# greatscottgadgets/libbtbb

Measured on AMD Instinct MI355X. Metric: Gbit/s raw bitstream scanned (LAP_ANY, err<=2), higher is better.
Workload: dtype u64; 1 GPU; promiscuous LAP_ANY scan, 4 GiB packed single-channel synthetic bitstream per GPU, max_ac_errors=2, sync word every 4096 symbols; symbols_per_gpu=34359738305, hits_per_gpu=6402406, parallelism=time-sharded x1 (btbbx_shard_plan: slices + 63-symbol halo), no collectives

## Files before the change

libbtbb_amd/csrc/packet_trials.h:

```cpp
#pragma once


__device__ __forceinline__ uint32_t lds_now(const uint32_t *p)
{
	return *(volatile __attribute__((address_space(3))) const uint32_t *)p;
}

#define TL_THREADS 512
#define TL_PACKETS (TL_THREADS / 16)
#define TL_WGS_PER_CU (1024 / TL_THREADS)
#define TL_TRIALS  (TL_PACKETS * 64)
#define TL_A_BLOCKS 183
#define TL_A_BYTES  232
#define TL_B_BLOCKS 10
#define TL_B_BYTES  16
#ifdef TL_PROFILE
__device__ unsigned long long g_tl_prof[16];
#define TL_PROF_START __shared__ uint32_t tl_acc[16]; if (threadIdx.x < 16) tl_acc[threadIdx.x] = 0; uint64_t tl_t = __builtin_readcyclecounter()
#define TL_PROF(k) do { const uint64_t n_ = __builtin_readcyclecounter(); if (tid == 0) tl_acc[k] += (uint32_t)(n_ - tl_t); tl_t = n_; } while (0)
#define TL_PROF_END do { __syncthreads(); if (tid < 16) atomicAdd(&g_tl_prof[tid], (unsigned long long)tl_acc[tid]); } while (0)
#else
#define TL_PROF_START do { } while (0)
#define TL_PROF(k) do { } while (0)
#define TL_PROF_END do { } while (0)
#endif
#define TL_AFAIL(p) lds_now(&a_fail[p])
__global__ __launch_bounds__(TL_THREADS) __attribute__((amdgpu_waves_per_eu(4, 4))) void trials_linear_kernel(const uint64_t *packets, const btbbx_pkt_in *in,
							     uint32_t n_packets, btbbx_trial *trials, const uint32_t *d_count)
{
	if (d_count)
		n_packets = min(n_packets, *d_count);
	__shared__ uint64_t pk[TL_PACKETS][BTBBX_PKT_WORDS + 1];
	__shared__ __attribute__((aligned(8))) btbbx_pkt_in pin[TL_PACKETS];
	__shared__ uint32_t hdr_ut[TL_PACKETS];
	__shared__ uint16_t clk_ut[64];
	__shared__ __attribute__((aligned(16))) uint16_t pw20[64];
	__shared__ __attribute__((aligned(16))) uint16_t lin[LIN_MAXLEN * 16];
	__shared__ __attribute__((aligned(16))) uint16_t advw[7 * 2 * 256];
	__shared__ uint16_t order[TL_TRIALS];
	__shared__ uint32_t t_info[TL_TRIALS];
	__shared__ int16_t t_rv[TL_TRIALS];
	__shared__ uint32_t pk_sort[TL_PACKETS];
	__shared__ uint32_t type_base[18];
	__shared__ uint16_t a10[TL_PACKETS][TL_A_BLOCKS + 3];
	static_assert(TL_A_BYTES / 4 + LIN_MAXLEN / 4 <= TL_A_BLOCKS + 3, "p4a and p4c of a packet lie in its a10 row");
	__shared__ uint16_t b10[TL_PACKETS][TL_B_BLOCKS + 2];
	__shared__ uint32_t a_bytes[TL_PACKETS][TL_A_BYTES / 4], b_bytes[TL_PACKETS][TL_B_BYTES / 4];
	__shared__ uint32_t a_fail[TL_PACKETS], b_fail[TL_PACKETS];
	__shared__ uint16_t p4b[TL_PACKETS][TL_B_BYTES / 4];
	auto p4a = [&](uint32_t p) { return &a10[p][0]; };
	auto p4c = [&](uint32_t p) { return &a10[p][TL_A_BYTES / 4]; };
	__shared__ int8_t hv_rv[TL_PACKETS];
	__shared__ uint16_t chunk_reg[TL_PACKETS][20];
	const uint32_t tid = threadIdx.x, lane = tid & 63;
	TL_PROF_START;
	for (uint32_t i = tid; i < LIN_MAXLEN * 2; i += TL_THREADS)
		reinterpret_cast<uint4 *>(lin)[i] = reinterpret_cast<const uint4 *>(g_lin)[i];
	for (uint32_t i = tid; i < 7 * 2 * 256 / 8; i += TL_THREADS)
		reinterpret_cast<uint4 *>(advw)[i] = reinterpret_cast<const uint4 *>(g_advw)[i];
	chain_lds_init();
	if (tid >= 64 && tid < 128) {
		const uint32_t wb = (uint32_t)wh_bits(wh_start(tid - 64, 0), 18);
		const uint32_t wt = (wb >> 3) & 0xf;
		uint32_t crank = 0;
		for (uint32_t k = 0; k < 16; k++) {
			const uint64_t mk = __ballot(wt == k);
			if (wt == k)
				crank = __builtin_amdgcn_mbcnt_hi((uint32_t)(mk >> 32), __builtin_amdgcn_mbcnt_lo((uint32_t)mk, 0));
		}
		clk_ut[tid - 64] = (uint16_t)(uap_from_hec(wb & 0x3ff, wb >> 10) | (wt << 8) | (crank << 12));
		const uint32_t v = (uint32_t)wh_bits(wh_start(tid - 64, 18), 7);
		uint32_t x = 0;
		for (int j = 0; j < 7; j++)
			if ((v >> j) & 1)
				x ^= lin[20 * 16 + 8 + j];
		pw20[tid - 64] = (uint16_t)x;
	}
	const uint32_t n_batches = (n_packets + TL_PACKETS - 1) / TL_PACKETS;
	constexpr uint32_t PK_ELEMS = TL_PACKETS * (BTBBX_PKT_WORDS + 1), IN_ELEMS = TL_PACKETS * sizeof(btbbx_pkt_in) / 8;
	constexpr uint32_t PER_THREAD = (PK_ELEMS + IN_ELEMS + TL_THREADS - 1) / TL_THREADS;
	static_assert(sizeof(btbbx_pkt_in) == 16, "two words per btbbx_pkt_in");
	uint64_t pre[PER_THREAD];
	auto fetch = [&](uint32_t b) {
		const uint32_t f = b * TL_PACKETS, have = b < n_batches ? (n_packets - f < TL_PACKETS ? n_packets - f : TL_PACKETS) : 0;
		uint32_t tv = tid;
		asm volatile("" : "+v"(tv));
#pragma unroll
		for (uint32_t k = 0; k < PER_THREAD; k++) {
			const uint32_t i = tv + TL_THREADS * k;
			const uint32_t p = i / (BTBBX_PKT_WORDS + 1), w = i % (BTBBX_PKT_WORDS + 1), e = i - PK_ELEMS;
			const uint64_t *src = packets;
			if (i < PK_ELEMS) {
				if (p < have && w < BTBBX_PKT_WORDS)
					src = packets + (uint64_t)(f + p) * BTBBX_PKT_WORDS + w;
			} else if (e < 2 * have) {
				src = reinterpret_cast<const uint64_t *>(in) + (uint64_t)f * 2 + e;
			}
			pre[k] = *src;
		}
	};
	auto stage_in = [&](uint32_t b) {
		const uint32_t f = b * TL_PACKETS, have = b < n_batches ? (n_packets - f < TL_PACKETS ? n_packets - f : TL_PACKETS) : 0;
		uint32_t tv = tid;
		asm volatile("" : "+v"(tv));
#pragma unroll
		for (uint32_t k = 0; k < PER_THREAD; k++) {
			const uint32_t i = tv + TL_THREADS * k;
			const uint32_t p = i / (BTBBX_PKT_WORDS + 1), w = i % (BTBBX_PKT_WORDS + 1);
			if (i < PK_ELEMS)
				pk[p][w] = (p < have && w < BTBBX_PKT_WORDS) ? pre[k] : 0;
			else if (i < PK_ELEMS + IN_ELEMS)
				reinterpret_cast<uint64_t *>(pin)[i - PK_ELEMS] = pre[k];
		}
		if (tid < TL_PACKETS) {
			a_fail[tid] = TL_A_BLOCKS;
			b_fail[tid] = TL_B_BLOCKS;
		}
	};
	fetch(blockIdx.x);
	stage_in(blockIdx.x);
	fetch(blockIdx.x + gridDim.x);
	for (uint32_t batch = blockIdx.x; batch < n_batches; batch += gridDim.x) {
	const uint32_t first = batch * TL_PACKETS;
	const uint32_t mine = n_packets - first < TL_PACKETS ? n_packets - first : TL_PACKETS;

	__syncthreads();
	TL_PROF(0);

	static_assert(TL_PACKETS <= 64, "one wave ranks the packets of a batch");
	if (tid < 64) {
		const bool live = tid < mine;
		uint32_t h = 0;
		if (live) {
			uint32_t dis;
			const uint32_t hdr = header_fec13(pk[tid], dis);
			h = uap_from_hec(hdr & 0x3ff, hdr >> 10) | (((hdr >> 3) & 0xf) << 8) | ((dis < 4 ? 1u : 0u) << 16);
			hdr_ut[tid] = h;
		}
		const bool fec_ok = (h & 0x10000u) != 0;
		const bool var = live && fec_ok && (pin[live ? tid : 0].flags & F_WHITENED);
		const uint32_t key = !live ? 0u : fec_ok ? (h >> 8) & 0xfu : (uint32_t)pin[tid].type & 0xfu;
		const uint64_t vm = __ballot(var);
		const uint32_t nvar = (uint32_t)__popcll(vm);
		uint32_t rank = __builtin_amdgcn_mbcnt_hi((uint32_t)(vm >> 32), __builtin_amdgcn_mbcnt_lo((uint32_t)vm, 0));
		const bool fixed = live && !var;
		uint32_t cf = 0;
		if (__ballot(fixed)) {
			for (uint32_t k = 0; k < 16; k++) {
				const uint64_t fm = __ballot(fixed && key == k);
				if (fixed && key == k)
					rank = __builtin_amdgcn_mbcnt_hi((uint32_t)(fm >> 32), __builtin_amdgcn_mbcnt_lo((uint32_t)fm, 0));
				if (lane == k)
					cf = (uint32_t)__popcll(fm);
			}
		}
		uint32_t incl = cf;
#pragma unroll
		for (int dd = 1; dd < 16; dd <<= 1) {
			const uint32_t up = __shfl_up(incl, dd);
			if (lane >= (uint32_t)dd)
				incl += up;
		}
		if (lane < 16)
			type_base[lane] = 4u * nvar * lane + 64u * (incl - cf);
		if (lane == 17)
			type_base[17] = nvar;
		if (tid < TL_PACKETS)
			pk_sort[tid] = key | ((var ? 1u : 0u) << 4) | (rank << 8);
	}
	static_assert(TL_THREADS == 16 * TL_PACKETS, "sixteen threads per packet");
	auto a_words = [&](uint32_t p) {
		const uint32_t blocks = TL_AFAIL(p) < TL_A_BLOCKS ? TL_AFAIL(p) : TL_A_BLOCKS, n = (blocks * 10 + 31) / 32 + 1;
		return n < TL_A_BYTES / 4 ? n : (uint32_t)(TL_A_BYTES / 4);
	};
	{
		const uint32_t p = tid >> 4, sub = tid & 15;
		if (p < mine) {
			uint32_t d;
			if (sub < TL_B_BLOCKS) {
				if (!fec23_block(pk_bits32(pk[p], 202 + 15 * sub, 15), d))
					atomicMin(&b_fail[p], sub);
				b10[p][sub] = (uint16_t)d;
			}
#pragma unroll 1
			for (uint32_t k0 = 0; k0 < TL_A_BLOCKS; k0 += 16) {
				const uint32_t k = k0 + sub;
				if (k < TL_A_BLOCKS) {
					if (!fec23_block(pk_bits32(pk[p], 122 + 15 * k, 15), d))
						atomicMin(&a_fail[p], k);
					a10[p][k] = (uint16_t)d;
				}
				__builtin_amdgcn_fence(__ATOMIC_ACQ_REL, "wavefront");
				if (TL_AFAIL(p) < k0 + 16)
					break;
			}
			__builtin_amdgcn_fence(__ATOMIC_ACQ_REL, "wavefront");
			auto word_from = [&](const uint16_t *src, uint32_t nblk, uint32_t word) {
				const uint32_t bit = 32 * word, k0 = bit / 10, sh = bit % 10;
				uint64_t acc = 0;
				for (uint32_t j = 0; j < 5; j++)
					acc |= (uint64_t)(k0 + j < nblk ? src[k0 + j] : 0) << (10 * j);
				return (uint32_t)(acc >> sh);
			};
			if (sub < TL_B_BYTES / 4)
				b_bytes[p][sub] = word_from(b10[p], TL_B_BLOCKS, sub);
			const uint32_t need = a_words(p);
			for (uint32_t word = sub; word < need; word += 16)
				a_bytes[p][word] = word_from(a10[p], TL_A_BLOCKS, word);
		}
	}
	if (tid >= 128 && tid < 128 + mine) {
		const uint32_t p = tid - 128;
		int rv = 1;
		if ((int)pin[p].length - 122 >= 240) {
			uint32_t total = 0;
			for (int i = 0; i < 4; i++) {
				uint32_t dis;
				(void)fec13(pk_bits(pk[p], 122 + 60 * i, 60), 20, dis);
				total += dis;
			}
			rv = total < 20 ? 2 : 0;
		}
		hv_rv[p] = (int8_t)rv;
	}
	__syncthreads();
	TL_PROF(1);
	const uint32_t total = mine * 64;
	for (uint32_t i = tid; i < total; i += TL_THREADS) {
		const uint32_t p = i >> 6;
		const uint32_t h = hdr_ut[p];
		uint32_t uap = pin[p].uap, type = pin[p].type, ret = 0;
		const uint32_t ps = pk_sort[p], cu = clk_ut[lane];
		if (h & 0x10000u) {
			const uint32_t v = (h ^ ((pin[p].flags & F_WHITENED) ? (cu & 0xfffu) : 0u)) & 0xffff;
			uap = ret = v & 0xff;
			type = v >> 8;
		}
		t_info[i] = ret | (type << 8) | (uap << 16);
		const uint32_t slot = (ps & 0x10u) ? type_base[type & 15] + 4u * (ps >> 8) + (cu >> 12)
						   : type_base[type & 15] + 4u * type_base[17] + 64u * (ps >> 8) + lane;
		order[slot] = (uint16_t)i;
	}
	auto chunk_of = [&](uint32_t t, uint32_t &p, uint32_t &r, uint32_t &layout, uint32_t &j, uint32_t &nwords) {
		if (t < mine * 12) {
			p = t / 12;
			j = t % 12;
			if (j < 11) { layout = 0; r = j; nwords = j < 10 ? 8 : LIN_MAXLEN / 4 - 80; }
			else { layout = 2; r = 19; j = 0; nwords = TL_B_BYTES / 4; }
		} else {
			const uint32_t u = t - mine * 12;
			j = mine == TL_PACKETS ? u / TL_PACKETS : u / mine;
			p = u - j * mine;
			layout = 1;
			r = 11 + j;
			const uint32_t need = a_words(p);
			nwords = need > 8 * j ? (need - 8 * j < 8 ? need - 8 * j : 8) : 0;
		}
	};
	auto data_word = [&](uint32_t p, uint32_t layout, uint32_t i) {
		return layout == 0 ? pk_bits32(pk[p], 122 + 32 * i, 32) : layout == 1 ? a_bytes[p][i] : b_bytes[p][i];
	};
	auto chunk_words = [&](uint32_t p, uint32_t layout, uint32_t j, uint32_t nwords, uint32_t (&w8)[8]) {
		if (layout == 0) {
			const uint32_t *d = reinterpret_cast<const uint32_t *>(pk[p]) + 3 + 8 * j;
			uint32_t raw[9];
#pragma unroll
			for (uint32_t i = 0; i < 9; i++)
				raw[i] = i <= nwords ? d[i] : 0;
#pragma unroll
			for (uint32_t i = 0; i < 8; i++)
				w8[i] = __builtin_amdgcn_alignbit(raw[i + 1], raw[i], 26);
		} else {
#pragma unroll
			for (uint32_t i = 0; i < 8; i++)
				w8[i] = i < nwords ? data_word(p, layout, 8 * j + i) : 0;
		}
	};
	for (uint32_t t = tid; t < mine * 20; t += TL_THREADS) {
		uint32_t p, r, layout, j, nwords, crc = 0;
		chunk_of(t, p, r, layout, j, nwords);
		if (!nwords)
			continue;
		uint32_t w8[8];
		chunk_words(p, layout, j, nwords, w8);
		uint16_t *dst = layout == 0 ? p4c(p) : layout == 1 ? p4a(p) : p4b[p];
#pragma unroll
		for (uint32_t i = 0; i < 8; i++)
			if (i < nwords) {
				dst[8 * j + i] = (uint16_t)crc;
				crc = crc_word(crc, w8[i]);
			}
		chunk_reg[p][r] = (uint16_t)crc;
	}
	__syncthreads();
	TL_PROF(8);
	if (tid >= 64 && tid < 64 + 3 * mine) {
		const uint32_t p = (tid - 64) / 3, layout = (tid - 64) % 3;
		const uint32_t r0 = layout == 0 ? 0 : layout == 1 ? 11 : 19;
		const uint32_t n = layout == 0 ? 11 : layout == 1 ? (a_words(p) + 7) / 8 : 1;
		uint32_t start = 0;
		for (uint32_t j = 0; j < n; j++) {
			const uint32_t c = chunk_reg[p][r0 + j];
			chunk_reg[p][r0 + j] = (uint16_t)start;
			start = g_lds.adv32[0][start & 0xff] ^ g_lds.adv32[1][start >> 8] ^ c;
		}
	}
	__syncthreads();
	TL_PROF(4);

	for (uint32_t kk = tid; kk < total; kk += TL_THREADS) {
		const uint32_t i = order[kk], p = i >> 6, clock = i & 63;
		const uint32_t info = t_info[i], type = (info >> 8) & 0xff, uap = (info >> 16) & 0xff;
		const bool wht = pin[p].flags & F_WHITENED;
		const int size = (int)pin[p].length - 122;
		const uint32_t seed = crc_seed(uap);
		const uint32_t sel = (seed >> 8) | (wht ? (uint32_t)wh_bits(wh_start(clock, 18), 7) << 8 : 0u);
		auto seed_row20 = [&](uint32_t sd) {
			const uint4 r0 = reinterpret_cast<const uint4 *>(lin)[40];
			const uint32_t r[4] = {r0.x, r0.y, r0.z, r0.w};
			uint32_t x = 0;
#pragma unroll
			for (int bit = 0; bit < 8; bit++)
				x ^= (0u - ((sd >> (8 + bit)) & 1)) & (r[bit >> 1] >> (16 * (bit & 1)));
			return x & 0xffff;
		};
		auto lin_terms = [&](uint32_t L) {
			uint32_t x = 0;
#pragma unroll
			for (int half = 0; half < 2; half++) {
				const uint4 q = reinterpret_cast<const uint4 *>(lin)[2 * L + half];
				const uint32_t r[4] = {q.x, q.y, q.z, q.w};
				const uint32_t sl = sel >> (8 * half);
#pragma unroll
				for (int bit = 0; bit < 8; bit++)
					x ^= (0u - ((sl >> bit) & 1)) & (r[bit >> 1] >> (16 * (bit & 1)));
			}
			return x & 0xffff;
		};
		auto data_reg = [&](int layout, uint32_t L) {
			const uint32_t q = L >> 2, r = L & 3;
			uint32_t crc, w;
			if (layout == 0) { crc = p4c(p)[q]; w = r ? pk_bits32(pk[p], 122 + 32 * q, 32) : 0; }
			else if (layout == 1) { crc = p4a(p)[q]; w = r ? a_bytes[p][q] : 0; }
			else { crc = p4b[p][q]; w = r ? b_bytes[p][q] : 0; }
			const uint32_t start = chunk_reg[p][(layout == 0 ? 0u : layout == 1 ? 11u : 19u) + (q >> 3)], iw = q & 7;
			crc ^= iw ? (uint32_t)(advw[((iw - 1) * 2) * 256 + (start & 0xff)] ^ advw[((iw - 1) * 2 + 1) * 256 + (start >> 8)]) : start;
			for (uint32_t j = 0; j < r; j++)
				crc = crc_byte(crc, (w >> (8 * j)) & 0xff);
			return crc;
		};
		auto crc_is_zero = [&](int layout, uint32_t L) {
			return (data_reg(layout, L) ^ lin_terms(L)) == 0;
		};
		int rv = 1;
		switch (type) {
		case 2: {
			if (size < 240) { rv = 1; break; }
			if (a_fail[p] < 16) { rv = 0; break; }
			const uint32_t x = data_reg(1, 20) ^ seed_row20(seed);
			rv = 0;
			if (!wht) {
				if (x == 0) rv = 1000;
			} else {
				uint32_t hit = x == pw20[clock];
				const uint32_t xx = x | (x << 16);
#pragma unroll 1
				for (int v = 0; v < 4; v++) {
					const uint4 q = reinterpret_cast<const uint4 *>(&pw20[32])[v];
					const uint32_t d0 = q.x ^ xx, d1 = q.y ^ xx, d2 = q.z ^ xx, d3 = q.w ^ xx;
					hit |= ((d0 & 0xffff) == 0) | ((d0 >> 16) == 0) | ((d1 & 0xffff) == 0) | ((d1 >> 16) == 0)
					     | ((d2 & 0xffff) == 0) | ((d2 >> 16) == 0) | ((d3 & 0xffff) == 0) | ((d3 >> 16) == 0);
				}
				if (hit) rv = 1000;
			}
			break;
		}
		case 3: case 8: case 10: case 14:
		case 4: case 11: case 15: {
			const bool fec = type == 3 || type == 8 || type == 10 || type == 14;
			const int layout = !fec ? 0 : (type == 8 ? 2 : 1);
			const int psize = type == 8 ? size - 80 : size;
			const int hb = (type == 3 || type == 8 || type == 4) ? 1 : 2;
			const int hbits = 8 * hb;
			const uint32_t fail = layout == 2 ? b_fail[p] : a_fail[p];
			rv = 0;
			if (psize < hbits) break;
			uint32_t raw;
			if (fec) {
				if (psize < (hb == 2 ? 30 : 15)) break;
				if (fail < (uint32_t)hb) break;
				raw = (layout == 2 ? b_bytes[p][0] : a_bytes[p][0]) & ((1u << hbits) - 1);
			} else {
				raw = pk_bits32(pk[p], 122, hbits);
			}
			const uint32_t ph = raw ^ (wht ? (uint32_t)wh_bits(wh_start(clock, 18), hbits) : 0u);
			int plen = hb == 2 ? (int)((ph >> 3) & 0x3ff) + 4 : (int)((ph >> 3) & 0x1f) + 3;
			int cap;
			switch (type) {
			case 3:  cap = 20;  break;
			case 4:  cap = 30;  break;
			case 8:  cap = 12;  break;
			case 10: cap = 125; break;
			case 11: cap = 187; break;
			case 14: cap = 228; break;
			default: cap = 343; break;
			}
			if (plen > cap) plen = cap;
			const int nbits = plen * 8;
			if (nbits > psize) { rv = 1; break; }
			if (fec && fail < (uint32_t)(nbits + 9) / 10) break;
			rv = crc_is_zero(layout, (uint32_t)plen) ? 10 : 2;
			break;
		}
		case 12: {
			uint32_t B = size >= 15 ? (uint32_t)size / 15 : 0;
			if (B > 98) B = 98;
			if (B > a_fail[p]) B = a_fail[p];
			const uint32_t lmax = B ? 5 * (B - 1) / 4 : 0;
			uint32_t crc = seed, idx = wh_start(clock, 18);
			rv = B == 98 ? 2 : 1;
			for (uint32_t L0 = 0; L0 < lmax; L0 += 4) {
				const uint32_t w = a_bytes[p][L0 >> 2] ^ (wht ? (uint32_t)wh_bits(idx, 32) : 0u);
				idx = idx + 32 >= 127 ? idx + 32 - 127 : idx + 32;
				const uint32_t x0 = (crc ^ w) & 0xff, x1 = ((crc ^ w) >> 8) & 0xff, b2 = (w >> 16) & 0xff, b3 = w >> 24;
				const uint32_t c1 = (crc >> 8) ^ g_lds.crc[x0];
				const uint32_t c2 = g_lds.crc_z[0][x0] ^ g_lds.crc[x1];
				const uint32_t c3 = g_lds.crc_z[1][x0] ^ g_lds.crc_z[0][x1] ^ g_lds.crc[b2];
				const uint32_t c4 = g_lds.crc_z[2][x0] ^ g_lds.crc_z[1][x1] ^ g_lds.crc_z[0][b2] ^ g_lds.crc[b3];
				const bool z1 = c1 == 0 && L0 + 1 >= 2 && L0 + 1 <= lmax, z2 = c2 == 0 && L0 + 2 <= lmax;
				const bool z3 = c3 == 0 && L0 + 3 <= lmax, z4 = c4 == 0 && L0 + 4 <= lmax;
				if (z1 || z2 || z3 || z4) { rv = 10; break; }
				crc = c4;
			}
			break;
		}
		case 5: rv = hv_rv[p]; break;
		default: rv = 1; break;
		}
		if (rv == 0 && type != 2 && type != 3 && type != 5)
			rv = 1;
		t_rv[i] = (int16_t)rv;
	}
	__syncthreads();
	TL_PROF(5);
	stage_in(batch + gridDim.x);
	fetch(batch + 2 * gridDim.x);
	static_assert(sizeof(btbbx_trial) == 4, "one dword per trial");
	for (uint32_t i = tid; i < total; i += TL_THREADS)
		reinterpret_cast<uint32_t *>(trials)[(uint64_t)first * 64 + i] =
			(t_info[i] & 0xffff) | ((uint32_t)(uint16_t)t_rv[i] << 16);
	TL_PROF(6);
	}
	TL_PROF_END;
}

__global__ __launch_bounds__(64) void trials_wide_kernel(const uint64_t *packets, const btbbx_pkt_in *in,
							  uint32_t n_packets, btbbx_trial *trials, const uint32_t *d_count)
{
	chain_lds_init();
	if (d_count)
		n_packets = min(n_packets, *d_count);
	const uint32_t pkt = blockIdx.x >> 6, clock = blockIdx.x & 63;
	if (threadIdx.x || pkt >= n_packets)
		return;
	const btbbx_pkt_in pi = in[pkt];
	PState s;
	s.w = packets + (uint64_t)pkt * BTBBX_PKT_WORDS;
	s.length = (int)pi.length;
	pstate_enter(s, pi);
	pstate_blank_out(s);
	uint32_t dis;
	const uint32_t hdr = header_fec13(s.w, dis);
	const uint32_t uap = do_try_clock(s, clock, hdr, dis);
	const int rv = do_crc_check<false>(s, clock);
	btbbx_trial t;
	t.uap = (uint8_t)uap;
	t.type = (uint8_t)s.type;
	t.rv = (int16_t)rv;
	trials[(uint64_t)pkt * 64 + clock] = t;
}

__global__ __launch_bounds__(256) void uap_table_kernel(const uint64_t *packets, const btbbx_pkt_in *in, uint32_t n,
							 uint4 *table)
{
	const uint32_t lane = threadIdx.x & 63;
	const uint32_t pkt0 = (blockIdx.x * 4 + (threadIdx.x >> 6)) * 64;
	if (pkt0 >= n)
		return;
	uint32_t ut = 0;
	if (pkt0 + lane < n) {
		const uint32_t p = pkt0 + lane;
		uint32_t dis;
		const uint32_t hdr = fec13((packets[(uint64_t)p * BTBBX_PKT_WORDS + 1] >> 4) & ((1ULL << 54) - 1), 18, dis);
		const uint32_t wht = in ? (in[p].flags & F_WHITENED) : 1u;
		ut = uap_from_hec(hdr & 0x3ff, hdr >> 10) | (((hdr >> 3) & 0xf) << 8) | ((dis < 4 ? 1u : 0u) << 16) | (wht << 17);
	}
	uint32_t wc[4] = {0, 0, 0, 0};
#pragma unroll
	for (int k = 0; k < 8; k++) {
		const uint32_t wb = (uint32_t)wh_bits_const(wh_start_const(8 * (lane & 7) + k, 0), 18);
		const uint32_t e = uap_from_hec(wb & 0x3ff, wb >> 10) | (((wb >> 3) & 0xf) << 8);
		wc[k >> 1] |= e << (16 * (k & 1));
	}
#pragma unroll
	for (int j = 0; j < 8; j++) {
		const uint32_t src = 8 * j + (lane >> 3);
		const uint32_t v = (uint32_t)__shfl((int)ut, (int)src);
		const uint32_t both = (v & 0xffff) * 0x10001u;
		const uint32_t okm = 0u - ((v >> 16) & 1u), whm = 0u - ((v >> 17) & 1u);
		uint4 o;
		o.x = (both ^ (wc[0] & whm)) & okm;
		o.y = (both ^ (wc[1] & whm)) & okm;
		o.z = (both ^ (wc[2] & whm)) & okm;
		o.w = (both ^ (wc[3] & whm)) & okm;
		if (pkt0 + src < n)
			table[(uint64_t)(pkt0 + src) * 8 + (lane & 7)] = o;
	}
}
```

Baseline: 12800 Gbit/s.

## Shrink LDS footprint and raise trials kernel occupancy to three workgroups per CU

```diff
diff --git a/libbtbb_amd/csrc/packet_trials.h b/libbtbb_amd/csrc/packet_trials.h
--- a/libbtbb_amd/csrc/packet_trials.h
+++ b/libbtbb_amd/csrc/packet_trials.h
@@ -8,7 +8,8 @@
 
 #define TL_THREADS 512
 #define TL_PACKETS (TL_THREADS / 16)
-#define TL_WGS_PER_CU (1024 / TL_THREADS)
+#define TL_WGS_PER_CU 3
+#define TL_WAVES_PER_EU (TL_WGS_PER_CU * TL_THREADS / 256)
 #define TL_TRIALS  (TL_PACKETS * 64)
 #define TL_A_BLOCKS 183
 #define TL_A_BYTES  232
@@ -25,7 +26,7 @@
 #define TL_PROF_END do { } while (0)
 #endif
 #define TL_AFAIL(p) lds_now(&a_fail[p])
-__global__ __launch_bounds__(TL_THREADS) __attribute__((amdgpu_waves_per_eu(4, 4))) void trials_linear_kernel(const uint64_t *packets, const btbbx_pkt_in *in,
+__global__ __launch_bounds__(TL_THREADS) __attribute__((amdgpu_waves_per_eu(TL_WAVES_PER_EU, TL_WAVES_PER_EU))) void trials_linear_kernel(const uint64_t *packets, const btbbx_pkt_in *in,
 							     uint32_t n_packets, btbbx_trial *trials, const uint32_t *d_count)
 {
 	if (d_count)
@@ -35,27 +36,23 @@
 	__shared__ uint32_t hdr_ut[TL_PACKETS];
 	__shared__ uint16_t clk_ut[64];
 	__shared__ __attribute__((aligned(16))) uint16_t pw20[64];
-	__shared__ __attribute__((aligned(16))) uint16_t lin[LIN_MAXLEN * 16];
 	__shared__ __attribute__((aligned(16))) uint16_t advw[7 * 2 * 256];
 	__shared__ uint16_t order[TL_TRIALS];
-	__shared__ uint32_t t_info[TL_TRIALS];
-	__shared__ int16_t t_rv[TL_TRIALS];
+	__shared__ uint8_t rv8[TL_TRIALS];
 	__shared__ uint32_t pk_sort[TL_PACKETS];
 	__shared__ uint32_t type_base[18];
 	__shared__ uint16_t a10[TL_PACKETS][TL_A_BLOCKS + 3];
-	static_assert(TL_A_BYTES / 4 + LIN_MAXLEN / 4 <= TL_A_BLOCKS + 3, "p4a and p4c of a packet lie in its a10 row");
+	static_assert(TL_A_BYTES / 4 + LIN_MAXLEN / 4 + 20 + TL_B_BYTES / 4 <= TL_A_BLOCKS + 3, "p4a, p4c, chunk_reg and p4b of a packet lie in its a10 row");
 	__shared__ uint16_t b10[TL_PACKETS][TL_B_BLOCKS + 2];
 	__shared__ uint32_t a_bytes[TL_PACKETS][TL_A_BYTES / 4], b_bytes[TL_PACKETS][TL_B_BYTES / 4];
 	__shared__ uint32_t a_fail[TL_PACKETS], b_fail[TL_PACKETS];
-	__shared__ uint16_t p4b[TL_PACKETS][TL_B_BYTES / 4];
 	auto p4a = [&](uint32_t p) { return &a10[p][0]; };
 	auto p4c = [&](uint32_t p) { return &a10[p][TL_A_BYTES / 4]; };
+	auto chunk_reg = [&](uint32_t p) { return &a10[p][TL_A_BYTES / 4 + LIN_MAXLEN / 4]; };
+	auto p4b = [&](uint32_t p) { return &a10[p][TL_A_BYTES / 4 + LIN_MAXLEN / 4 + 20]; };
 	__shared__ int8_t hv_rv[TL_PACKETS];
-	__shared__ uint16_t chunk_reg[TL_PACKETS][20];
-	const uint32_t tid = threadIdx.x, lane = tid & 63;
+	const uint32_t tid = threadIdx.x;
 	TL_PROF_START;
-	for (uint32_t i = tid; i < LIN_MAXLEN * 2; i += TL_THREADS)
-		reinterpret_cast<uint4 *>(lin)[i] = reinterpret_cast<const uint4 *>(g_lin)[i];
 	for (uint32_t i = tid; i < 7 * 2 * 256 / 8; i += TL_THREADS)
 		reinterpret_cast<uint4 *>(advw)[i] = reinterpret_cast<const uint4 *>(g_advw)[i];
 	chain_lds_init();
@@ -73,15 +70,14 @@
 		uint32_t x = 0;
 		for (int j = 0; j < 7; j++)
 			if ((v >> j) & 1)
-				x ^= lin[20 * 16 + 8 + j];
+				x ^= g_lin[20 * 16 + 8 + j];
 		pw20[tid - 64] = (uint16_t)x;
 	}
 	const uint32_t n_batches = (n_packets + TL_PACKETS - 1) / TL_PACKETS;
 	constexpr uint32_t PK_ELEMS = TL_PACKETS * (BTBBX_PKT_WORDS + 1), IN_ELEMS = TL_PACKETS * sizeof(btbbx_pkt_in) / 8;
 	constexpr uint32_t PER_THREAD = (PK_ELEMS + IN_ELEMS + TL_THREADS - 1) / TL_THREADS;
 	static_assert(sizeof(btbbx_pkt_in) == 16, "two words per btbbx_pkt_in");
-	uint64_t pre[PER_THREAD];
-	auto fetch = [&](uint32_t b) {
+	auto fetch = [&](uint32_t b, uint64_t (&pre)[PER_THREAD]) {
 		const uint32_t f = b * TL_PACKETS, have = b < n_batches ? (n_packets - f < TL_PACKETS ? n_packets - f : TL_PACKETS) : 0;
 		uint32_t tv = tid;
 		asm volatile("" : "+v"(tv));
@@ -99,7 +95,7 @@
 			pre[k] = *src;
 		}
 	};
-	auto stage_in = [&](uint32_t b) {
+	auto stage_in = [&](uint32_t b, const uint64_t (&pre)[PER_THREAD]) {
 		const uint32_t f = b * TL_PACKETS, have = b < n_batches ? (n_packets - f < TL_PACKETS ? n_packets - f : TL_PACKETS) : 0;
 		uint32_t tv = tid;
 		asm volatile("" : "+v"(tv));
@@ -117,10 +113,16 @@
 			b_fail[tid] = TL_B_BLOCKS;
 		}
 	};
-	fetch(blockIdx.x);
-	stage_in(blockIdx.x);
-	fetch(blockIdx.x + gridDim.x);
+	{
+		uint64_t w0[PER_THREAD];
+		fetch(blockIdx.x, w0);
+		stage_in(blockIdx.x, w0);
+	}
+	const uint32_t tid0 = tid;
 	for (uint32_t batch = blockIdx.x; batch < n_batches; batch += gridDim.x) {
+	uint32_t tid = tid0;
+	asm volatile("" : "+v"(tid));
+	const uint32_t lane = tid & 63;
 	const uint32_t first = batch * TL_PACKETS;
 	const uint32_t mine = n_packets - first < TL_PACKETS ? n_packets - first : TL_PACKETS;
 
@@ -226,17 +228,24 @@
 	__syncthreads();
 	TL_PROF(1);
 	const uint32_t total = mine * 64;
-	for (uint32_t i = tid; i < total; i += TL_THREADS) {
+	auto trial_info = [&](uint32_t p, uint32_t clock) {
+		const uint32_t h = hdr_ut[p];
+		if (!(h & 0x10000u))
+			return ((uint32_t)pin[p].type << 8) | ((uint32_t)pin[p].uap << 16);
+		const uint32_t v = (h ^ ((pin[p].flags & F_WHITENED) ? (clk_ut[clock] & 0xfffu) : 0u)) & 0xffff;
+		return v | ((v & 0xff) << 16);
+	};
+	static_assert(TL_TRIALS == 4 * TL_THREADS, "four trials per thread");
+	uint32_t out_lo[2] = {0, 0};
+#pragma unroll
+	for (uint32_t k = 0; k < 4; k++) {
+		const uint32_t i = tid + TL_THREADS * k;
+		if (i >= total)
+			break;
 		const uint32_t p = i >> 6;
-		const uint32_t h = hdr_ut[p];
-		uint32_t uap = pin[p].uap, type = pin[p].type, ret = 0;
+		const uint32_t info = trial_info(p, lane), type = (info >> 8) & 0xff;
+		out_lo[k >> 1] |= (info & 0xffff) << (16 * (k & 1));
 		const uint32_t ps = pk_sort[p], cu = clk_ut[lane];
-		if (h & 0x10000u) {
-			const uint32_t v = (h ^ ((pin[p].flags & F_WHITENED) ? (cu & 0xfffu) : 0u)) & 0xffff;
-			uap = ret = v & 0xff;
-			type = v >> 8;
-		}
-		t_info[i] = ret | (type << 8) | (uap << 16);
 		const uint32_t slot = (ps & 0x10u) ? type_base[type & 15] + 4u * (ps >> 8) + (cu >> 12)
 						   : type_base[type & 15] + 4u * type_base[17] + 64u * (ps >> 8) + lane;
 		order[slot] = (uint16_t)i;
@@ -283,14 +292,14 @@
 			continue;
 		uint32_t w8[8];
 		chunk_words(p, layout, j, nwords, w8);
-		uint16_t *dst = layout == 0 ? p4c(p) : layout == 1 ? p4a(p) : p4b[p];
+		uint16_t *dst = layout == 0 ? p4c(p) : layout == 1 ? p4a(p) : p4b(p);
 #pragma unroll
 		for (uint32_t i = 0; i < 8; i++)
 			if (i < nwords) {
 				dst[8 * j + i] = (uint16_t)crc;
 				crc = crc_word(crc, w8[i]);
 			}
-		chunk_reg[p][r] = (uint16_t)crc;
+		chunk_reg(p)[r] = (uint16_t)crc;
 	}
 	__syncthreads();
 	TL_PROF(8);
@@ -300,8 +309,8 @@
 		const uint32_t n = layout == 0 ? 11 : layout == 1 ? (a_words(p) + 7) / 8 : 1;
 		uint32_t start = 0;
 		for (uint32_t j = 0; j < n; j++) {
-			const uint32_t c = chunk_reg[p][r0 + j];
-			chunk_reg[p][r0 + j] = (uint16_t)start;
+			const uint32_t c = chunk_reg(p)[r0 + j];
+			chunk_reg(p)[r0 + j] = (uint16_t)start;
 			start = g_lds.adv32[0][start & 0xff] ^ g_lds.adv32[1][start >> 8] ^ c;
 		}
 	}
@@ -310,13 +319,13 @@
 
 	for (uint32_t kk = tid; kk < total; kk += TL_THREADS) {
 		const uint32_t i = order[kk], p = i >> 6, clock = i & 63;
-		const uint32_t info = t_info[i], type = (info >> 8) & 0xff, uap = (info >> 16) & 0xff;
+		const uint32_t info = trial_info(p, clock), type = (info >> 8) & 0xff, uap = (info >> 16) & 0xff;
 		const bool wht = pin[p].flags & F_WHITENED;
 		const int size = (int)pin[p].length - 122;
 		const uint32_t seed = crc_seed(uap);
 		const uint32_t sel = (seed >> 8) | (wht ? (uint32_t)wh_bits(wh_start(clock, 18), 7) << 8 : 0u);
 		auto seed_row20 = [&](uint32_t sd) {
-			const uint4 r0 = reinterpret_cast<const uint4 *>(lin)[40];
+			const uint4 r0 = reinterpret_cast<const uint4 *>(g_lin)[40];
 			const uint32_t r[4] = {r0.x, r0.y, r0.z, r0.w};
 			uint32_t x = 0;
 #pragma unroll
@@ -328,7 +337,7 @@
 			uint32_t x = 0;
 #pragma unroll
 			for (int half = 0; half < 2; half++) {
-				const uint4 q = reinterpret_cast<const uint4 *>(lin)[2 * L + half];
+				const uint4 q = reinterpret_cast<const uint4 *>(g_lin)[2 * L + half];
 				const uint32_t r[4] = {q.x, q.y, q.z, q.w};
 				const uint32_t sl = sel >> (8 * half);
 #pragma unroll
@@ -342,8 +351,8 @@
 			uint32_t crc, w;
 			if (layout == 0) { crc = p4c(p)[q]; w = r ? pk_bits32(pk[p], 122 + 32 * q, 32) : 0; }
 			else if (layout == 1) { crc = p4a(p)[q]; w = r ? a_bytes[p][q] : 0; }
-			else { crc = p4b[p][q]; w = r ? b_bytes[p][q] : 0; }
-			const uint32_t start = chunk_reg[p][(layout == 0 ? 0u : layout == 1 ? 11u : 19u) + (q >> 3)], iw = q & 7;
+			else { crc = p4b(p)[q]; w = r ? b_bytes[p][q] : 0; }
+			const uint32_t start = chunk_reg(p)[(layout == 0 ? 0u : layout == 1 ? 11u : 19u) + (q >> 3)], iw = q & 7;
 			crc ^= iw ? (uint32_t)(advw[((iw - 1) * 2) * 256 + (start & 0xff)] ^ advw[((iw - 1) * 2 + 1) * 256 + (start >> 8)]) : start;
 			for (uint32_t j = 0; j < r; j++)
 				crc = crc_byte(crc, (w >> (8 * j)) & 0xff);
@@ -439,16 +448,23 @@
 		}
 		if (rv == 0 && type != 2 && type != 3 && type != 5)
 			rv = 1;
-		t_rv[i] = (int16_t)rv;
+		rv8[i] = (uint8_t)(rv == 1000 ? 255 : rv);
 	}
 	__syncthreads();
 	TL_PROF(5);
-	stage_in(batch + gridDim.x);
-	fetch(batch + 2 * gridDim.x);
+	uint64_t nx[PER_THREAD];
+	fetch(batch + gridDim.x, nx);
 	static_assert(sizeof(btbbx_trial) == 4, "one dword per trial");
-	for (uint32_t i = tid; i < total; i += TL_THREADS)
+#pragma unroll
+	for (uint32_t k = 0; k < 4; k++) {
+		const uint32_t i = tid + TL_THREADS * k;
+		if (i >= total)
+			break;
+		const uint32_t c = rv8[i];
 		reinterpret_cast<uint32_t *>(trials)[(uint64_t)first * 64 + i] =
-			(t_info[i] & 0xffff) | ((uint32_t)(uint16_t)t_rv[i] << 16);
+			((out_lo[k >> 1] >> (16 * (k & 1))) & 0xffff) | ((c == 255 ? 1000u : c) << 16);
+	}
+	stage_in(batch + gridDim.x, nx);
 	TL_PROF(6);
 	}
 	TL_PROF_END;
```

Result: no change. 12800 Gbit/s (-0.0%).
